# z430/keyword-spotting

Measured on AMD Instinct MI355X. Metric: 1s 16kHz clips/sec end-to-end (wav->label), higher is better.
Workload: dtype f32

## Files before the change

### keyword-spotting_amd/csrc/kws_dscnn.hip

```cpp
#include <array>
#include <utility>

#include "kws_dscnn_stages.h"

namespace kws {
namespace {

#ifndef KWS_X_DSCNN_STAMP_TID
#define KWS_X_DSCNN_STAMP_TID 0
#endif

__device__ __forceinline__ DscnnWeights weights_for_this_clip() {
#if defined(__HIP_DEVICE_COMPILE__)
    using KArg = const __attribute__((address_space(4))) DscnnWeights*;
    KArg p = (KArg)__builtin_amdgcn_kernarg_segment_ptr();
    asm volatile("" : "+s"(p));
    return *p;
#else
    return DscnnWeights{};
#endif
}

using FwdKernelFn = void (*)(DscnnWeights, const float*, int, float*, int32_t*, float*, unsigned long long*, const int*, StreamPush);
struct FwdKernelArgs {
// ... 58 lines not shown
        if (i < IN_T * IN_F) featp[(i / IN_F + 2) * FEAT_W + (i % IN_F) + 2] = fv[k];
    }
    if constexpr (PAIR) {
        float m = 0.f;
#pragma unroll
        for (int k = 0; k < FV; ++k) m = fmaxf(m, fabsf(fv[k]));
        publish_wave_max(lds, 0, wv, lane, m);
        if (lane == 63) lds[OFF_WMAX + wv + STAGE_WAVES] = 0.f;
    }
}

__device__ __forceinline__ void pool_fc_wave(const DscnnWeights& w, const float* lds, int lane, int clip, float* __restrict__ logits,
                                             int32_t* __restrict__ label, float* __restrict__ a_pool) {
    const int C = w.num_classes;
    float4 fcw[CH / 4];
    float fcb = 0.f;
    const float4* wr = reinterpret_cast<const float4*>(w.fc_w + (lane < C ? lane : 0) * CH);
#pragma unroll
    for (int c = 0; c < CH / 4; ++c) fcw[c] = wr[c];
    if (lane < C) fcb = w.fc_b[lane];
    const float ring_b = w.pw_b[3 * CH + lane];
    constexpr float RING_N = 55.f * 11.f - 53.f * 9.f;
    float s = 0.f;
#pragma unroll
    for (int k = 0; k < NW; ++k) s += lds[OFF_POOLBUF_P + k * CH + lane];
    s = fmaf(RING_N, relu(ring_b), s) * (1.0f / (55.f * 11.f));
    if (a_pool) a_pool[lane] = s;
    float acc = fcb;
#pragma unroll
    for (int c = 0; c < CH / 4; ++c) {
        const float4 a4 = fcw[c];
        acc = fmaf(a4.x, __builtin_bit_cast(float, __builtin_amdgcn_readlane(__builtin_bit_cast(int, s), 4 * c + 0)), acc);
        acc = fmaf(a4.y, __builtin_bit_cast(float, __builtin_amdgcn_readlane(__builtin_bit_cast(int, s), 4 * c + 1)), acc);
        acc = fmaf(a4.z, __builtin_bit_cast(float, __builtin_amdgcn_readlane(__builtin_bit_cast(int, s), 4 * c + 2)), acc);
        acc = fmaf(a4.w, __builtin_bit_cast(float, __builtin_amdgcn_readlane(__builtin_bit_cast(int, s), 4 * c + 3)), acc);
    }
    if (lane < C) logits[(size_t)clip * C + lane] = acc;
    const int idx = wave_argmax_first(lane < C ? acc : -INFINITY, lane, C);
    if (label && lane == 0) label[clip] = idx;
}

template <int MODE, bool DIAG = true, bool PRECONV = false, bool STREAM = false, bool CLUSTER = false, bool PERSIST = false,
          bool SCAN = false>
__global__ __launch_bounds__(NT) void kws_dscnn_fwd_kernel(DscnnWeights w_arg, const float* __restrict__ feat, int B,
                                                           float* __restrict__ logits, int32_t* __restrict__ label,
                                                           float* __restrict__ act_arg,
                                                           unsigned long long* __restrict__ stamps_arg,
                                                           const int* __restrict__ ring_hops, StreamPush sp) {
    static_assert(!STREAM || (MODE >= 4 && !DIAG && !PRECONV), "the fused push exists for the product paths only");
    static_assert(!PERSIST || ((MODE == 4 || MODE == 5) && !PRECONV && !STREAM), "persistent workgroups: batched product paths only");
    static_assert(!SCAN || ((MODE == 4 || MODE == 5) && !DIAG && !PRECONV && !STREAM && !CLUSTER), "strided windows: batched product paths only");
    constexpr bool PAIR = MODE == 5;
    constexpr int NP = PAIR ? 2 : 3;
    BlockTables t1_pre{};
    static_assert(!CLUSTER || STREAM, "time-tile clusters exist for the streaming push only");
    float* const act = DIAG ? act_arg : nullptr;
    unsigned long long* const stamps = DIAG ? stamps_arg : nullptr;
    extern __shared__ __attribute__((aligned(16))) float lds[];
    constexpr bool MFMA = MODE != 0;
    const int tid_k = threadIdx.x;
    const int lane_k = tid_k & 63, wv_k = tid_k >> 6;

    const int cl_n = CLUSTER ? sp.cluster : 1;
    int clip = CLUSTER ? (int)blockIdx.x / cl_n : (int)blockIdx.x;
    const int cl_tile = CLUSTER ? (int)blockIdx.x - clip * cl_n : 0;
    if (clip >= B) return;
    const int j0 = Blk<4>::H * cl_tile / cl_n, j1 = Blk<4>::H * (cl_tile + 1) / cl_n;
    auto rows = [&](int lo, int hi, int H, int W) { return PosRange{(lo < 0 ? 0 : lo) * W, (hi > H ? H : hi) * W}; };
    const PosRange rg4 = rows(j0, j1, Blk<4>::H, Blk<4>::W), rg3 = rows(j0 - 2, j1, Blk<3>::H, Blk<3>::W),
                   rg2 = rows(j0 - 4, j1, Blk<2>::H, Blk<2>::W), rg1 = rows(j0 - 6, j1, Blk<1>::H, Blk<1>::W),
                   rg0 = rows(j0 - 7, j1 + 1, C1_H, C1_W);
    int n_stamp = 0;
    auto stamp = [&]() {
        if (stamps && tid_k == KWS_X_DSCNN_STAMP_TID) stamps[(size_t)clip * KWS_DSCNN_STAMPS + n_stamp] = __builtin_amdgcn_s_memtime();
        ++n_stamp;
    };

    constexpr bool SPLIT = MODE >= 4;
    constexpr bool UT = PERSIST && PAIR;
    BlockTables t1p{};
    uintx4 c1p[PERSIST ? 7 : 1][NP];
    int prev_clip = -1;
    float* a_prev = nullptr;
    if constexpr (PERSIST) {
        fetch_block_tables(w_arg, 1, tid_k, t1p);
        if (wv_k < STAGE_WAVES) stage_features_persist<PAIR, SCAN>(lds, feat, clip, tid_k, sp.scan);
        load_conv1_frags(w_arg, wv_k, lane_k, c1p);
        __syncthreads();
    }
    for (;;) {
    auto weights_now = [&]() -> DscnnWeights { return PERSIST ? weights_for_this_clip() : w_arg; };
    const DscnnWeights w = weights_now();
    int tid = tid_k;
    if constexpr (PERSIST) {
        int wv_l = __builtin_amdgcn_readfirstlane(wv_k), lane_l = lane_k;
        asm volatile("" : "+s"(wv_l), "+v"(lane_l));
        tid = (wv_l << 6) | (lane_l & 63);
    }
    const int lane = tid & 63, wv = tid >> 6;
    if constexpr (PERSIST) n_stamp = 0;
    if (stamps && tid == KWS_X_DSCNN_STAMP_TID) stamps[(size_t)clip * KWS_DSCNN_STAMPS + KWS_DSCNN_STAMPS - 2] = __builtin_amdgcn_s_memrealtime();
    stamp();

    PwOperands<MODE> wa;
    UnitDesc ud{};
    int hops_before = 0;
    int kx = 0, ky[5] = {0, 0, 0, 0, 0}, sg[5] = {0, 0, 0, 0, 0};
    if constexpr (PERSIST) {
        if constexpr (PAIR) {
            const float mxf = read_stage_max(lds, 0, 1);
            kx = pow2_exp_for(mxf);
            const float bz0 = (w.c1_abs * mxf + w.c1_bmax) * 1.001f;
            cap_units(kx, sg[0], w.k_c1, bz0);
            const float by1 = (w.dw_abs[0] * bz0 + w.dw_bmax[0]) * 1.001f;
            ky[1] = pow2_exp_for(by1);
            cap_units(ky[1], sg[1], w.k_pw[0], (w.pw_abs[0] * by1 + w.pw_bmax[0]) * 1.001f);
            store_block_tables(lds, 1, tid, t1p, pow2f(ky[1]), pow2f(sg[1]), pow2f(ky[1] - sg[0]));
            conv1_build_windows(lds, tid, pow2f(kx), OFF_FEAT_P);
            __syncthreads();
        } else {
            store_block_tables(lds, 1, tid, t1p);
        }
        stamp();
        conv1_phase_split<false, NP>(w, lds, tid, c1p, rg0, pow2f(kx), pow2f(sg[0]), OFF_FEAT_P);
        if (wv == NW - 1 && prev_clip >= 0) {
            pool_fc_wave(w, lds, lane, prev_clip, logits, label, a_prev);
            if (stamps && lane == 0) stamps[(size_t)prev_clip * KWS_DSCNN_STAMPS + 13] = __builtin_amdgcn_s_memtime();
        }
        if constexpr (UT) load_unit_desc(w, 1, wv < Leftover<1>::TILE ? wv : Leftover<1>::TILE, lane, ud);
        load_afrag(w, 1, wv >= 4 ? wv - 4 : 0, lane, wa.ring[0]);
    } else if constexpr (PRECONV) {
        static_assert(!PRECONV || MODE >= 4, "the pre-convolved entry exists for the product (split) path only");
        const float* z = feat + (size_t)clip * (CH * P0);
        fetch_block_tables(w, 1, tid, t1_pre);
        float zmax = 0.f;
        for (int i = tid; i < CH * P0; i += NT) {
            const float v = z[i];
            lds[OFF_Z0 + pidx(i / P0, i % P0, P0 + 2)] = v;
            zmax = fmaxf(zmax, v);
        }
        if (tid < CH) {
            lds[OFF_Z0 + pidx(tid, P0, P0 + 2)] = 0.f;
            lds[OFF_Z0 + pidx(tid, P0 + 1, P0 + 2)] = 0.f;
        }
        if constexpr (PAIR)
            publish_wave_max(lds, 1, wv, lane, zmax);
        else
            store_block_tables(lds, 1, tid, t1_pre);
        if constexpr (Leftover<1>::HAS && (MODE == 4 || MODE == 5) && !CLUSTER)
            load_afrag(w, 1, wv >= 4 ? wv - 4 : 0, lane, wa.ring[0]);
        else
            load_block_head(w, 1, lane, wa);
        stamp();
    } else {
    float* featp = lds + OFF_FEAT;
    const float* f = clip_features<SCAN>(feat, clip, sp.scan);
    constexpr int FV = (IN_T * IN_F + NT - 1) / NT;
    float fv[FV];
    int row_new = -1;
    int head;
    if constexpr (STREAM) {
        hops_before = *sp.hops;
        const int K = frames_lag(sp.p);
        head = (((hops_before + 2 - K) % IN_T) + IN_T) % IN_T;
        const int step = sp.p.frame_step;
        const long f_start = (long)step * hops_before + step - (long)K * step;
// ... 12 lines not shown
    float a1[SPLIT ? 1 : 50];
    uintx4 c1f[SPLIT ? 7 : 1][NP];
    if constexpr (SPLIT) {
        load_conv1_frags(w, wv, lane, c1f);
    } else if constexpr (MFMA) {
        const int half = lane >> 5, col = lane & 31, ct = wv & 1;
#pragma unroll
        for (int s = 0; s < 50; ++s) a1[s] = w.c1_w[(2 * s + half) * CH + ct * 32 + col];
        load_pointwise(w, 1, lane, wa);
    }
    __builtin_amdgcn_sched_barrier(0);
    if constexpr (PAIR) {
        float m = 0.f;
#pragma unroll
        for (int k = 0; k < FV; ++k) m = fmaxf(m, fabsf(fv[k]));
        publish_wave_max(lds, 0, wv, lane, m);
    }
    if constexpr (STREAM) {
#ifdef KWS_X_STREAM_NO_FRAME
        if (false)
#else
        if (wv == 0 && cl_tile == cl_n - 1)
#endif
            stream_frame_wave(sp.p, sp.t, sp.hop, clip, clip, false, sp.pcm_ring, sp.ring_len, const_cast<float*>(feat), hops_before,
                              reinterpret_cast<unsigned char*>(lds + OFF_Z2), lane,
                              row_new >= 0 ? featp + (row_new + 2) * FEAT_W + 2 : nullptr, sp.refine_ctr);
        for (int i = tid; i < FEAT_H * FEAT_W; i += NT) {
            const int r = i / FEAT_W - 2, c = i % FEAT_W - 2;
            if (!((unsigned)r < (unsigned)IN_T && (unsigned)c < (unsigned)IN_F)) featp[i] = 0.f;
        }
        if constexpr (!PAIR) store_block_tables(lds, 1, tid, t1);
#pragma unroll
        for (int k = 0; k < FV; ++k) {
            const int i = tid + k * NT;
            if (i < IN_T * IN_F && i / IN_F != row_new) featp[(i / IN_F + 2) * FEAT_W + (i % IN_F) + 2] = fv[k];
        }
        __syncthreads();
    } else {
    for (int i = tid; i < FEAT_H * FEAT_W; i += NT) {
        const int r = i / FEAT_W - 2, c = i % FEAT_W - 2;
        if (!((unsigned)r < (unsigned)IN_T && (unsigned)c < (unsigned)IN_F)) featp[i] = 0.f;
    }
    if constexpr (!PAIR) store_block_tables(lds, 1, tid, t1);
#pragma unroll
    for (int k = 0; k < FV; ++k) {
        const int i = tid + k * NT;
        if (i < IN_T * IN_F) featp[(i / IN_F + 2) * FEAT_W + (i % IN_F) + 2] = fv[k];
    }
    __syncthreads();
    }
    if constexpr (PAIR) {
        float mxf = read_stage_max(lds, 0, 1);
        if constexpr (STREAM) {
            if (row_new >= 0 && cl_tile == cl_n - 1)
                for (int c = 0; c < IN_F; ++c) mxf = fmaxf(mxf, fabsf(featp[(row_new + 2) * FEAT_W + 2 + c]));
        }
        kx = pow2_exp_for(mxf);
        const float bz0 = (w.c1_abs * mxf + w.c1_bmax) * 1.001f;
        cap_units(kx, sg[0], w.k_c1, bz0);
        const float by1 = (w.dw_abs[0] * bz0 + w.dw_bmax[0]) * 1.001f;
        ky[1] = pow2_exp_for(by1);
        cap_units(ky[1], sg[1], w.k_pw[0], (w.pw_abs[0] * by1 + w.pw_bmax[0]) * 1.001f);
        store_block_tables(lds, 1, tid, t1, pow2f(ky[1]), pow2f(sg[1]), pow2f(ky[1] - sg[0]));
        conv1_build_windows(lds, tid, pow2f(kx));
        __syncthreads();
    }
    stamp();

    if constexpr (SPLIT) {
        conv1_phase_split<CLUSTER, NP>(w, lds, tid, c1f, rg0, pow2f(kx), pow2f(sg[0]));
        if constexpr (Leftover<1>::HAS && (MODE == 4 || MODE == 5) && !CLUSTER)
            load_afrag(w, 1, wv >= 4 ? wv - 4 : 0, lane, wa.ring[0]);
        else
            load_block_head(w, 1, lane, wa);
    } else {
        conv1_phase<MFMA>(w, lds, tid, a1);
    }
    }
    stamp();
    const DscnnWeights w1 = weights_now();
    __syncthreads();
    stamp();
    float* a = act ? act + (size_t)clip * KWS_ACT_FLOATS_PER_CLIP : nullptr;
    constexpr bool KSL_ON = (MODE == 4 || MODE == 5) && !CLUSTER;
    if (a) {
        const float u = PAIR ? pow2f(-sg[0]) : 1.f;
        for (int i = tid; i < CH * P0; i += NT) a[i] = lds[OFF_Z0 + pidx(i / P0, i % P0, P0 + 2)] * u;
        a += CH * P0;
    }
    PairCtx pc;
    if constexpr (PAIR && PRECONV) {
        const float mz0 = read_stage_max(lds, 1, 1);
        const float by1 = (w1.dw_abs[0] * mz0 + w1.dw_bmax[0]) * 1.001f;
        ky[1] = pow2_exp_for(by1);
        cap_units(ky[1], sg[1], w1.k_pw[0], (w1.pw_abs[0] * by1 + w1.pw_bmax[0]) * 1.001f);
        store_block_tables(lds, 1, tid, t1_pre, pow2f(ky[1]), pow2f(sg[1]), pow2f(ky[1]));
        __syncthreads();
    }
    if constexpr (PAIR) {
        const float mz = read_stage_max(lds, 1, 1) * pow2f(-sg[0]);
        const float bz = (w1.pw_abs[0] * ((w1.dw_abs[0] * mz + w1.dw_bmax[0]) * 1.001f) + w1.pw_bmax[0]) * 1.001f;
        const float by = (w1.dw_abs[1] * bz + w1.dw_bmax[1]) * 1.001f;
        ky[2] = pow2_exp_for(by);
        cap_units(ky[2], sg[2], w1.k_pw[1], (w1.pw_abs[1] * by + w1.pw_bmax[1]) * 1.001f);
        pc.s_dww = pow2f(ky[2] - sg[1]);
        pc.s_dwb = pow2f(ky[2]);
        pc.s_pwb = pow2f(sg[2]);
    }
    block_phase<1, MODE, CLUSTER, UT>(w1, lds, tid, wa, ud, nullptr, rg1, pc);
    stamp();
    const DscnnWeights w2 = weights_now();
    __syncthreads();
    if constexpr (Leftover<1>::HAS && KSL_ON) {
        leftover_combine<1, PAIR>(lds, tid);
        __syncthreads();
    }
    stamp();
    if (a) {
        const float u = PAIR ? pow2f(-sg[1]) : 1.f;
        for (int i = tid; i < CH * Blk<1>::POUT; i += NT)
            a[i] = lds[OFF_Z1 + pidx(i / Blk<1>::POUT, i % Blk<1>::POUT, Blk<1>::SOUT)] * u;
        a += CH * Blk<1>::POUT;
    }
    if constexpr (PAIR) {
        const float mz = fmaxf(read_stage_max(lds, 2, (Leftover<1>::HAS && KSL_ON) ? 2 : 1) * pow2f(-sg[1]), w2.pw_bmax[0]);
        const float bz = (w2.pw_abs[1] * ((w2.dw_abs[1] * mz + w2.dw_bmax[1]) * 1.001f) + w2.pw_bmax[1]) * 1.001f;
        const float by = (w2.dw_abs[2] * bz + w2.dw_bmax[2]) * 1.001f;
        ky[3] = pow2_exp_for(by);
        cap_units(ky[3], sg[3], w2.k_pw[2], (w2.pw_abs[2] * by + w2.pw_bmax[2]) * 1.001f);
        pc.s_dww = pow2f(ky[3] - sg[2]);
        pc.s_dwb = pow2f(ky[3]);
        pc.s_pwb = pow2f(sg[3]);
    }
    block_phase<2, MODE, CLUSTER, UT>(w2, lds, tid, wa, ud, nullptr, rg2, pc);
    stamp();
    const DscnnWeights w3 = weights_now();
    __syncthreads();
    if constexpr (Leftover<2>::HAS && KSL_ON) {
        leftover_combine<2, PAIR>(lds, tid);
        __syncthreads();
    }
    stamp();
    if (a) {
        const float u = PAIR ? pow2f(-sg[2]) : 1.f;
        for (int i = tid; i < CH * Blk<2>::POUT; i += NT)
            a[i] = lds[OFF_Z2 + pidx(i / Blk<2>::POUT, i % Blk<2>::POUT, Blk<2>::SOUT)] * u;
        a += CH * Blk<2>::POUT;
    }
    if constexpr (PAIR) {
        const float mz = fmaxf(read_stage_max(lds, 0, (Leftover<2>::HAS && KSL_ON) ? 2 : 1) * pow2f(-sg[2]), w3.pw_bmax[1]);
        const float bz = (w3.pw_abs[2] * ((w3.dw_abs[2] * mz + w3.dw_bmax[2]) * 1.001f) + w3.pw_bmax[2]) * 1.001f;
        const float by = (w3.dw_abs[3] * bz + w3.dw_bmax[3]) * 1.001f;
        ky[4] = pow2_exp_for(by);
        cap_units(ky[4], sg[4], w3.k_pw[3], (w3.pw_abs[3] * by + w3.pw_bmax[3]) * 1.001f);
        pc.s_dww = pow2f(ky[4] - sg[3]);
        pc.s_dwb = pow2f(ky[4]);
        pc.s_pwb = pow2f(sg[4]);
    }
    block_phase<3, MODE, CLUSTER, UT>(w3, lds, tid, wa, ud, nullptr, rg3, pc);
    stamp();
    const DscnnWeights w4 = weights_now();
    __syncthreads();
    stamp();
    if (a) {
        const float u = PAIR ? pow2f(-sg[3]) : 1.f;
        for (int i = tid; i < CH * Blk<3>::POUT; i += NT)
            a[i] = lds[OFF_Z3 + pidx(i / Blk<3>::POUT, i % Blk<3>::POUT, Blk<3>::SOUT)] * u;
        a += CH * Blk<3>::POUT;
    }
    if constexpr (PAIR) {
        pc.inv_out = pow2f(-sg[4]);
    }
    block_phase<4, MODE, CLUSTER, UT>(w4, lds, tid, wa, ud, a ? a + CH : nullptr, rg4, pc,
                                      PERSIST ? OFF_POOLBUF_P : OFF_POOLBUF);
    stamp();
    if constexpr (PERSIST) {
        const int next = clip + (int)gridDim.x;
        __builtin_amdgcn_sched_barrier(0);
        const ScanWindows sw_next = SCAN ? scan_windows_now() : ScanWindows{};
        if (wv < STAGE_WAVES && next < B) stage_features_persist<PAIR, SCAN>(lds, feat, next, tid, sw_next);
        stamp();
        load_conv1_frags(w4, wv, lane, c1p);
        __syncthreads();
        stamp();
        if (stamps && tid == KWS_X_DSCNN_STAMP_TID) stamps[(size_t)clip * KWS_DSCNN_STAMPS + KWS_DSCNN_STAMPS - 1] = __builtin_amdgcn_s_memrealtime();
        prev_clip = clip;
        a_prev = a;
        clip = next;
        if (clip >= B) break;
        continue;
    }
    const int C = w4.num_classes;
    float4 fcw[CH / 4];
    float fcb = 0.f, ring_b = 0.f;
    if (wv == 0 && lane < C) {
        const float4* wr = reinterpret_cast<const float4*>(w4.fc_w + lane * CH);
#pragma unroll
        for (int c = 0; c < CH / 4; ++c) fcw[c] = wr[c];
        fcb = w4.fc_b[lane];
    }
    if (tid < CH) ring_b = w4.pw_b[3 * CH + tid];
    __syncthreads();
    stamp();

    float* pooled = lds + OFF_POOLED;
    constexpr float RING_N = 55.f * 11.f - 53.f * 9.f;
    bool run_fc = true;
    if constexpr (CLUSTER) {
        float* part = sp.cl_part + ((size_t)clip * cl_n + cl_tile) * CH;
        if (tid < CH) {
            float s = 0.f;
#pragma unroll
            for (int k = 0; k < NW; ++k) s += lds[OFF_POOLBUF + k * CH + tid];
            __hip_atomic_store(part + tid, s, __ATOMIC_RELAXED, __HIP_MEMORY_SCOPE_AGENT);
        }
        asm volatile("s_waitcnt vmcnt(0)" ::: "memory");
        __syncthreads();
        int* last_flag = reinterpret_cast<int*>(lds + OFF_POOLED + CH);
        if (tid == 0) {
            const int arrived = atomicAdd(&sp.cl_count[clip], 1);
            *last_flag = arrived == cl_n - 1;
            if (arrived == cl_n - 1) sp.cl_count[clip] = 0;
        }
        __syncthreads();
        run_fc = *last_flag != 0;
        if (run_fc) {
            if (tid < CH) {
                float s = 0.f;
                for (int t = 0; t < cl_n; ++t)
                    s += __hip_atomic_load(sp.cl_part + ((size_t)clip * cl_n + t) * CH + tid, __ATOMIC_RELAXED, __HIP_MEMORY_SCOPE_AGENT);
                pooled[tid] = fmaf(RING_N, relu(ring_b), s) * (1.0f / (55.f * 11.f));
            }
        }
// ... 162 lines not shown
```

### keyword-spotting_amd/csrc/kws_dscnn_geom.h

```cpp
#pragma once
#include "kws_internal.h"

namespace kws {
namespace {

#ifndef KWS_DSCNN_WAVES
#define KWS_DSCNN_WAVES 8
#endif
constexpr int NW = KWS_DSCNN_WAVES;
constexpr int NT = NW * 64;
constexpr int TW = 30;

constexpr int P0 = C1_H * C1_W;
constexpr int FEAT_H = 103, FEAT_W = 14;
constexpr int OFF_Z3 = 0, OFF_Z2 = 22976, OFF_Z1 = 0, OFF_Z0 = 9152, OFF_FEAT = 18304;
constexpr int OFF_DWTAB = 38784;
constexpr int OFF_PWB = OFF_DWTAB + 2 * 768;
constexpr int OFF_POOLED = OFF_PWB + 2 * 64;
constexpr int OFF_POOLBUF = OFF_DWTAB;
constexpr int OFF_WMAX = OFF_POOLED + 64 + 8;
constexpr int LDS_FLOATS = 40960;
static_assert(OFF_WMAX + 4 * NW <= LDS_FLOATS, "LDS overflow");
static_assert(NW * 64 <= 768, "pool scratch must fit one depthwise buffer");
static_assert(OFF_FEAT + FEAT_H * FEAT_W <= OFF_Z2, "feature pad overlaps Z2");
static_assert(CH * 12 <= 2 * NT, "table staging assumes at most two elements per thread");

__host__ __device__ __forceinline__ constexpr int pidx(int c, int p, int S) { return (c >> 1) * 2 * S + 2 * p + (c & 1); }

template <int N>
struct Blk {
    static constexpr int H = 45 + 2 * N, W = 1 + 2 * N;
    static constexpr bool RING = N > 1;
    static constexpr int HI = RING ? H - 2 : H, WI = RING ? W - 2 : W;
    static constexpr int PIN = HI * WI, SIN = PIN + 2;
    static constexpr int POUT = H * W, SOUT = POUT + 2;
    static constexpr int OFF_IN = N == 1 ? OFF_Z0 : N == 2 ? OFF_Z1 : N == 3 ? OFF_Z2 : OFF_Z3;
    static constexpr int OFF_OUT = N == 1 ? OFF_Z1 : N == 2 ? OFF_Z2 : OFF_Z3;
    static constexpr int TILES = (POUT + TW - 1) / TW;
    static constexpr int BUF = (N - 1) & 1;
};

#ifndef KWS_DSCNN_KSPLIT_LEFTOVER
#define KWS_DSCNN_KSPLIT_LEFTOVER 1
#endif
template <int N>
struct Leftover {
    static constexpr bool HAS = KWS_DSCNN_KSPLIT_LEFTOVER && (N == 1 || N == 2);
    static constexpr int TILE = N == 1 ? 4 : 8;
    static constexpr int P0T = TILE * TW;
    static constexpr int NP = HAS ? Blk<N>::POUT - P0T : 1;
    static constexpr int WAVE0 = N == 1 ? 4 : 0;
    static constexpr int OFF_PART = N == 1 ? OFF_Z2 : OFF_Z0;
};
static_assert(Blk<1>::TILES == 5 && Blk<2>::TILES == 9, "the leftover tiles are the fifth of block 1 and the ninth of block 2");
static_assert(4 * CH * Leftover<1>::NP <= 38784 - OFF_Z2 && OFF_Z0 + 4 * CH * Leftover<2>::NP <= OFF_FEAT, "partial sums fit their dead planes");

constexpr int OFF_FEAT_P = OFF_Z2;
constexpr int OFF_POOLBUF_P = OFF_FEAT_P + 1456;
constexpr int STAGE_WAVES = 4;
static_assert(OFF_FEAT_P >= OFF_Z3 + Blk<3>::SOUT * CH, "the next clip's features must not overlap block 4's input");
static_assert(OFF_FEAT_P + FEAT_H * FEAT_W <= OFF_POOLBUF_P && OFF_POOLBUF_P % 4 == 0, "features and pool partials are disjoint");
static_assert(OFF_POOLBUF_P + NW * CH <= OFF_Z2 + Blk<2>::SOUT * CH && OFF_Z2 + Blk<2>::SOUT * CH <= OFF_DWTAB,
              "pool partials stay inside the Z2 plane, clear of the table buffers the next clip's block 1 rewrites");

}
}
```

### keyword-spotting_amd/csrc/kws_dscnn_stages.h

```cpp
#pragma once
#include <type_traits>

#include "kws_dscnn_geom.h"
#include "kws_dscnn_units.h"
#include "kws_mfcc_dev.h"
#include "kws_split_mfma.h"

namespace kws {
namespace {

template <bool TO_MFMA = false>
__device__ __forceinline__ float stencil3x3(float w0, float w1, float w2, float w3, float w4, float w5, float w6,
                                            float w7, float w8, float b, float up, float mid, float dn, float mask_l,
                                            float mask_r) {
    float c, to_right, to_left;
    asm("v_mul_f32 %1, %3, %13\n\t"
        "v_mul_f32 %2, %5, %13\n\t"
        "v_fma_f32 %0, %4, %13, %12\n\t"
        "v_fmac_f32 %1, %6, %14\n\t"
        "v_fmac_f32 %2, %8, %14\n\t"
        "v_fmac_f32 %0, %7, %14\n\t"
        "v_fmac_f32 %1, %9, %15\n\t"
        "v_fmac_f32 %2, %11, %15\n\t"
        "v_fmac_f32 %0, %10, %15\n\t"
// ... 420 lines not shown
            conv1_unit_pairwin<true>(w, lds, z0, wv, wv & 1, lane, c1f, 0, P0, sig0, mx);
        else if (wv < 6)
            conv1_unit_pairwin<false>(w, lds, z0, 4, wv & 1, lane, c1f, 0, P0, sig0, mx);
    } else if constexpr (RANGED) {
        const int n_pt = (rg.hi - rg.lo + 31) / 32;
        for (int u = wv; u < 2 * n_pt; u += NW) conv1_unit_split<false, NP>(w, featp, z0, u >> 1, u & 1, lane, c1f, rg.lo, rg.hi, sx, sig0, mx);
    } else if (wv < 4)
        conv1_unit_split<true, NP>(w, featp, z0, wv, wv & 1, lane, c1f, 0, P0, sx, sig0, mx);
    else if (wv < 6)
        conv1_unit_split<false, NP>(w, featp, z0, 4, wv & 1, lane, c1f, 0, P0, sx, sig0, mx);
    if constexpr (NP == 2) publish_wave_max(lds, 1, wv, lane, mx);
    if (tid < CH) {
        z0[pidx(tid, P0, P0 + 2)] = 0.f;
        z0[pidx(tid, P0 + 1, P0 + 2)] = 0.f;
    }
}

template <int N, int NP, bool UT = false>
__device__ __forceinline__ void leftover_partial_unit(float* lds, int lane, int M, const uintx4 (&af)[2][NP], const UnitDesc& ud) {
    using G = Blk<N>;
    using L = Leftover<N>;
    const int half = lane >> 5, col = lane & 31;
    const float* dwtab = lds + OFF_DWTAB + G::BUF * 768;
    const float4* dwt4 = reinterpret_cast<const float4*>(dwtab) + half * 24;
    bool valid;
    float mask_l, mask_r;
    int ta[3];
    if constexpr (UT) {
        valid = ud.a[3] != 0u;
        mask_l = __builtin_bit_cast(float, ud.m.x), mask_r = __builtin_bit_cast(float, ud.m.y);
#pragma unroll
        for (int i = 0; i < 3; ++i) ta[i] = (int)ud.a[i];
    } else {
        const int pos = L::P0T - 1 + col;
        valid = col >= 1 && col <= TW && pos < G::POUT;
        const int posc = pos < G::POUT ? pos : G::POUT - 1;
        const int h = posc / G::W, x = posc % G::W;
        mask_l = x > 0 ? 1.f : 0.f, mask_r = x < G::W - 1 ? 1.f : 0.f;
#pragma unroll
        for (int dh = -1; dh <= 1; ++dh) {
            const int o = G::RING ? 1 : 0;
            const int hh = h + dh - o, xx = x - o;
            const bool inside = (unsigned)hh < (unsigned)G::HI && (unsigned)xx < (unsigned)G::WI;
            const bool in_map = (unsigned)(h + dh) < (unsigned)G::H;
            const int a = inside ? hh * G::WI + xx : ((G::RING && in_map) ? G::PIN : G::PIN + 1);
            ta[dh + 1] = G::OFF_IN + pidx(half * 8, a, G::SIN);
        }
    }
    float y[8];
#pragma unroll
    for (int j = 0; j < 8; j += 2) {
        const int cs = 16 * M + j;
        const int o = cs * G::SIN;
        const float2 up = *reinterpret_cast<const float2*>(lds + ta[0] + o);
        const float2 mid = *reinterpret_cast<const float2*>(lds + ta[1] + o);
        const float2 dn = *reinterpret_cast<const float2*>(lds + ta[2] + o);
        DwPair wp;
#pragma unroll
        for (int i = 0; i < 5; ++i) wp.l[i] = dwt4[(cs >> 1) * 6 + i];
        y[j] = stencil3x3_of_pair<false, 0>(wp, up.x, mid.x, dn.x, mask_l, mask_r);
        y[j + 1] = stencil3x3_of_pair<false, 1>(wp, up.y, mid.y, dn.y, mask_l, mask_r);
    }
    floatx16 acc0 = {0, 0, 0, 0, 0, 0, 0, 0, 0, 0, 0, 0, 0, 0, 0, 0}, acc1 = acc0;
    if constexpr (NP == 2) {
        uintx4 bh, bl;
        split_pair8_scaled(y, bh, bl);
        acc0 = mfma_f16(af[0][0], bl, acc0);
        acc1 = mfma_f16(af[1][0], bl, acc1);
        acc0 = mfma_f16(af[0][1], bh, acc0);
        acc1 = mfma_f16(af[1][1], bh, acc1);
        acc0 = mfma_f16(af[0][0], bh, acc0);
        acc1 = mfma_f16(af[1][0], bh, acc1);
    } else {
        uintx4 bh, bm, bl;
        split3(y, bh, bm, bl);
#pragma unroll
        for (int q = 0; q < 6; ++q) {
            const int pa = q == 0 ? 2 : (q == 2 || q == 3) ? 1 : 0;
            const uintx4& b = (q == 0 || q == 3 || q == 5) ? bh : (q == 1 ? bl : bm);
            acc0 = mfma_bf16(af[0][pa], b, acc0);
            acc1 = mfma_bf16(af[1][pa], b, acc1);
        }
    }
    float* part = lds + L::OFF_PART + M * (CH * L::NP);
    if (valid) {
#pragma unroll
        for (int r = 0; r < 16; ++r) {
            part[row_of(r, half) * L::NP + (col - 1)] = acc0[r];
            part[(32 + row_of(r, half)) * L::NP + (col - 1)] = acc1[r];
        }
    }
}

template <int N, bool PAIR = false>
__device__ __forceinline__ void leftover_combine(float* lds, int tid) {
    using G = Blk<N>;
    using L = Leftover<N>;
    const float* part = lds + L::OFF_PART;
    const float* pwb = lds + OFF_PWB + G::BUF * 64;
    float* zout = lds + G::OFF_OUT;
    float mx = 0.f;
    for (int i = tid; i < CH * L::NP; i += NT) {
        const int co = i / L::NP, j = i - co * L::NP;
        const float s = (part[i] + part[CH * L::NP + i]) + (part[2 * CH * L::NP + i] + part[3 * CH * L::NP + i]);
        const float v = relu(s + pwb[co]);
        zout[pidx(co, L::P0T + j, G::SOUT)] = v;
        mx = fmaxf(mx, v);
    }
    if constexpr (PAIR) publish_wave_max(lds, N == 1 ? 3 : 1, tid >> 6, tid & 63, mx);
}

template <int N, int MODE, bool RANGED = false, bool UT = false>
__device__ __forceinline__ void block_phase(const DscnnWeights& w, float* lds, int tid, PwOperands<MODE>& pwo, UnitDesc& ud,
                                            float* __restrict__ act4 = nullptr, PosRange rg = PosRange{0, 0}, PairCtx pc = PairCtx{},
                                            int off_poolbuf = OFF_POOLBUF) {
    static_assert(!UT || ((MODE == 4 || MODE == 5) && !RANGED && Leftover<1>::HAS), "unit descriptors: product paths on whole maps");
    using G = Blk<N>;
    constexpr bool PAIR = MODE == 5;
    constexpr int NP = PAIR ? 2 : 3;
    constexpr int NPROD = PAIR ? 3 : 6;
    constexpr bool KSL = Leftover<N>::HAS && (MODE == 4 || MODE == 5) && !RANGED;
    const int p_lo = RANGED ? rg.lo : 0, p_hi = RANGED ? rg.hi : G::POUT;
#ifdef KWS_X_DSCNN_SKIP_LEFTOVER
    const int n_tiles = RANGED ? (p_hi - p_lo + TW - 1) / TW : (N == 2 ? 8 : G::TILES);
#else
    const int n_tiles = RANGED ? (p_hi - p_lo + TW - 1) / TW : (KSL ? Leftover<N>::TILE : G::TILES);
#endif
    constexpr bool MFMA = MODE != 0;
    constexpr bool SPLIT = MODE >= 4;
    constexpr bool NO_STENCIL = MODE == 6;
    const int lane = tid & 63, wv = tid >> 6, half = lane >> 5, col = lane & 31;
    float* zout = lds + G::OFF_OUT;
    const float* dwtab = lds + OFF_DWTAB + G::BUF * 768;
    const float* pwb = lds + OFF_PWB + G::BUF * 64;
    float* poolbuf = lds + off_poolbuf;

    BlockTables next_tables;
    if constexpr (N < 4) {
        fetch_block_tables(w, N + 1, tid, next_tables);
        if (tid < CH) {
            zout[pidx(tid, G::POUT, G::SOUT)] = relu(pwb[tid]);
            zout[pidx(tid, G::POUT + 1, G::SOUT)] = 0.f;
        }
    } else if (!MFMA) {
        poolbuf[wv * CH + lane] = 0.f;
    }

    const float4* bias4 = reinterpret_cast<const float4*>(pwb) + half;
    const float4* dwt4 = reinterpret_cast<const float4*>(dwtab) + half * 24;
    float psum[2][16];
#pragma unroll
    for (int ct = 0; ct < 2; ++ct)
#pragma unroll
        for (int r = 0; r < 16; ++r) psum[ct][r] = 0.f;
    float stage_max = 0.f;

    for (int t = wv; t < n_tiles; t += NW) {
        const int pos = p_lo + t * TW - 1 + col;
        bool valid;
        uint32_t keep;
        float mask_l, mask_r;
        int tlo[3], thi[3];
        if constexpr (UT) {
            keep = ud.a[3];
            valid = keep != 0u;
            mask_l = __builtin_bit_cast(float, ud.m.x), mask_r = __builtin_bit_cast(float, ud.m.y);
#pragma unroll
            for (int i = 0; i < 3; ++i) {
                tlo[i] = (int)ud.a[i];
                thi[i] = tlo[i] + 32 * G::SIN;
                asm volatile("" : "+v"(tlo[i]));
                asm volatile("" : "+v"(thi[i]));
            }
        } else {
            valid = col >= 1 && col <= TW && pos < p_hi;
            keep = valid ? 0xffffffffu : 0u;
            const int posc = pos < p_lo ? p_lo : (pos < p_hi ? pos : p_hi - 1);
            const int h = posc / G::W, x = posc % G::W;
            mask_l = x > 0 ? 1.f : 0.f, mask_r = x < G::W - 1 ? 1.f : 0.f;
#pragma unroll
            for (int dh = -1; dh <= 1; ++dh) {
                const int o = G::RING ? 1 : 0;
                const int hh = h + dh - o, xx = x - o;
                const bool inside = (unsigned)hh < (unsigned)G::HI && (unsigned)xx < (unsigned)G::WI;
                const bool in_map = (unsigned)(h + dh) < (unsigned)G::H;
                const int a = inside ? hh * G::WI + xx : ((G::RING && in_map) ? G::PIN : G::PIN + 1);
                tlo[dh + 1] = G::OFF_IN + pidx(half * 8, a, G::SIN);
                thi[dh + 1] = tlo[dh + 1] + 32 * G::SIN;
                asm volatile("" : "+v"(tlo[dh + 1]));
                asm volatile("" : "+v"(thi[dh + 1]));
            }
        }
// ... 150 lines not shown
                        }
#pragma unroll
                        for (int r = 0; r < 16; r += 2) stage_max = fmaxf(stage_max, fmaxf(fmaxf(o0[r], o0[r + 1]), fmaxf(o1[r], o1[r + 1])));
                        if (valid) {
#pragma unroll
                            for (int r = 0; r < 16; r += 2) {
                                *reinterpret_cast<float2*>(zout + pidx(row_of(r, half), pos, G::SOUT)) = make_float2(o0[r], o0[r + 1]);
                                *reinterpret_cast<float2*>(zout + pidx(32 + row_of(r, half), pos, G::SOUT)) = make_float2(o1[r], o1[r + 1]);
                            }
                        }
                    } else if (valid) {
#pragma unroll
                        for (int r = 0; r < 16; r += 2) {
                            *reinterpret_cast<float2*>(zout + pidx(row_of(r, half), pos, G::SOUT)) =
                                make_float2(relu(acc0[r]), relu(acc0[r + 1]));
                            *reinterpret_cast<float2*>(zout + pidx(32 + row_of(r, half), pos, G::SOUT)) =
                                make_float2(relu(acc1[r]), relu(acc1[r + 1]));
                        }
                    }
                } else {
#pragma unroll
                    for (int r = 0; r < 16; ++r) {
                        psum[0][r] += __builtin_bit_cast(float, __builtin_bit_cast(uint32_t, relu(acc0[r])) & keep);
                        psum[1][r] += __builtin_bit_cast(float, __builtin_bit_cast(uint32_t, relu(acc1[r])) & keep);
                    }
                    if (act4 && valid) {
#pragma unroll
                        for (int r = 0; r < 16; ++r) {
                            act4[row_of(r, half) * G::POUT + pos] = relu(acc0[r]) * pc.inv_out;
                            act4[(32 + row_of(r, half)) * G::POUT + pos] = relu(acc1[r]) * pc.inv_out;
                        }
                    }
                }
            };
            if constexpr (!SPLIT) {
                if (N < 4 && t + NW >= n_tiles) {
                    __builtin_amdgcn_sched_barrier(0);
                    if constexpr (N < 4) load_pointwise(w, N + 1, lane, pwo);
                    __builtin_amdgcn_sched_barrier(0);
                    epilogue();
                    break;
                }
            }
            epilogue();
            if constexpr (UT) ud = ud_next;
        } else {
            const float* pw_w = w.pw_w + (N - 1) * CH * CH;
            float y[32];
#pragma unroll
            for (int s = 0; s < 32; s += 2) {
                TapPair tq;
                tap_pair_load(s >> 1, tq);
                DwPair wp;
                wts_pair_load(s >> 1, wp);
                y[s] = dw_eval(wp, tq, std::integral_constant<int, 0>{});
                y[s + 1] = dw_eval(wp, tq, std::integral_constant<int, 1>{});
            }
#pragma unroll 1
            for (int co = 0; co < CH; ++co) {
                float part = 0.f;
#pragma unroll
                for (int s = 0; s < 32; ++s) part = fmaf(pw_w[(16 * (s >> 3) + 8 * half + (s & 7)) * CH + co], y[s], part);
                const float tot = relu(part + __shfl_xor(part, 32, 64) + pwb[co]);
                if constexpr (N < 4) {
                    if (valid && half == 0) zout[pidx(co, pos, G::SOUT)] = tot;
                } else {
                    if (act4 && valid && half == 0) act4[co * G::POUT + pos] = tot;
                    float sum = (valid && half == 0) ? tot : 0.f;
#pragma unroll
                    for (int o = 16; o >= 1; o >>= 1) sum += __shfl_xor(sum, o, 64);
                    if (lane == 0) poolbuf[wv * CH + co] += sum;
                }
            }
        }
    }

    if constexpr (KSL) {
        using L = Leftover<N>;
        if (wv >= L::WAVE0 && wv < L::WAVE0 + 4) {
            leftover_partial_unit<N, NP, UT>(lds, lane, wv - L::WAVE0, pwo.ring[0], ud);
            __builtin_amdgcn_sched_barrier(0);
            if constexpr (UT) load_unit_desc(w, N + 1, wv, lane, ud);
            load_afrag(w, N + 1, 0, lane, pwo.ring[0]);
        }
    }
    if constexpr (N < 4) store_block_tables(lds, N + 1, tid, next_tables, pc.s_dwb, pc.s_pwb, pc.s_dww);
    if constexpr (PAIR && N <= 2) publish_wave_max(lds, N == 1 ? 2 : 0, wv, lane, stage_max);
    if constexpr (MFMA) {
        if constexpr (N < 4) {
            if (wv >= n_tiles && !(KSL && N == 1)) load_block_head(w, N + 1, lane, pwo);
        } else {
#pragma unroll
            for (int ct = 0; ct < 2; ++ct) {
                float (&q)[16] = psum[ct];
                asm volatile("s_nop 4\n\t"
                    "v_add_f32_dpp %0, %0, %0 row_shr:1 row_mask:0xf bank_mask:0xf bound_ctrl:1\n\t"
                    "v_add_f32_dpp %1, %1, %1 row_shr:1 row_mask:0xf bank_mask:0xf bound_ctrl:1\n\t"
                    "v_add_f32_dpp %2, %2, %2 row_shr:1 row_mask:0xf bank_mask:0xf bound_ctrl:1\n\t"
                    "v_add_f32_dpp %3, %3, %3 row_shr:1 row_mask:0xf bank_mask:0xf bound_ctrl:1\n\t"
                    "v_add_f32_dpp %4, %4, %4 row_shr:1 row_mask:0xf bank_mask:0xf bound_ctrl:1\n\t"
                    "v_add_f32_dpp %5, %5, %5 row_shr:1 row_mask:0xf bank_mask:0xf bound_ctrl:1\n\t"
                    "v_add_f32_dpp %6, %6, %6 row_shr:1 row_mask:0xf bank_mask:0xf bound_ctrl:1\n\t"
                    "v_add_f32_dpp %7, %7, %7 row_shr:1 row_mask:0xf bank_mask:0xf bound_ctrl:1\n\t"
                    "v_add_f32_dpp %8, %8, %8 row_shr:1 row_mask:0xf bank_mask:0xf bound_ctrl:1\n\t"
                    "v_add_f32_dpp %9, %9, %9 row_shr:1 row_mask:0xf bank_mask:0xf bound_ctrl:1\n\t"
                    "v_add_f32_dpp %10, %10, %10 row_shr:1 row_mask:0xf bank_mask:0xf bound_ctrl:1\n\t"
                    "v_add_f32_dpp %11, %11, %11 row_shr:1 row_mask:0xf bank_mask:0xf bound_ctrl:1\n\t"
                    "v_add_f32_dpp %12, %12, %12 row_shr:1 row_mask:0xf bank_mask:0xf bound_ctrl:1\n\t"
                    "v_add_f32_dpp %13, %13, %13 row_shr:1 row_mask:0xf bank_mask:0xf bound_ctrl:1\n\t"
                    "v_add_f32_dpp %14, %14, %14 row_shr:1 row_mask:0xf bank_mask:0xf bound_ctrl:1\n\t"
                    "v_add_f32_dpp %15, %15, %15 row_shr:1 row_mask:0xf bank_mask:0xf bound_ctrl:1\n\t"
                    "v_add_f32_dpp %0, %0, %0 row_shr:2 row_mask:0xf bank_mask:0xf bound_ctrl:1\n\t"
                    "v_add_f32_dpp %1, %1, %1 row_shr:2 row_mask:0xf bank_mask:0xf bound_ctrl:1\n\t"
                    "v_add_f32_dpp %2, %2, %2 row_shr:2 row_mask:0xf bank_mask:0xf bound_ctrl:1\n\t"
                    "v_add_f32_dpp %3, %3, %3 row_shr:2 row_mask:0xf bank_mask:0xf bound_ctrl:1\n\t"
                    "v_add_f32_dpp %4, %4, %4 row_shr:2 row_mask:0xf bank_mask:0xf bound_ctrl:1\n\t"
                    "v_add_f32_dpp %5, %5, %5 row_shr:2 row_mask:0xf bank_mask:0xf bound_ctrl:1\n\t"
                    "v_add_f32_dpp %6, %6, %6 row_shr:2 row_mask:0xf bank_mask:0xf bound_ctrl:1\n\t"
                    "v_add_f32_dpp %7, %7, %7 row_shr:2 row_mask:0xf bank_mask:0xf bound_ctrl:1\n\t"
                    "v_add_f32_dpp %8, %8, %8 row_shr:2 row_mask:0xf bank_mask:0xf bound_ctrl:1\n\t"
                    "v_add_f32_dpp %9, %9, %9 row_shr:2 row_mask:0xf bank_mask:0xf bound_ctrl:1\n\t"
                    "v_add_f32_dpp %10, %10, %10 row_shr:2 row_mask:0xf bank_mask:0xf bound_ctrl:1\n\t"
                    "v_add_f32_dpp %11, %11, %11 row_shr:2 row_mask:0xf bank_mask:0xf bound_ctrl:1\n\t"
                    "v_add_f32_dpp %12, %12, %12 row_shr:2 row_mask:0xf bank_mask:0xf bound_ctrl:1\n\t"
                    "v_add_f32_dpp %13, %13, %13 row_shr:2 row_mask:0xf bank_mask:0xf bound_ctrl:1\n\t"
                    "v_add_f32_dpp %14, %14, %14 row_shr:2 row_mask:0xf bank_mask:0xf bound_ctrl:1\n\t"
                    "v_add_f32_dpp %15, %15, %15 row_shr:2 row_mask:0xf bank_mask:0xf bound_ctrl:1\n\t"
                    "v_add_f32_dpp %0, %0, %0 row_shr:4 row_mask:0xf bank_mask:0xf bound_ctrl:1\n\t"
                    "v_add_f32_dpp %1, %1, %1 row_shr:4 row_mask:0xf bank_mask:0xf bound_ctrl:1\n\t"
                    "v_add_f32_dpp %2, %2, %2 row_shr:4 row_mask:0xf bank_mask:0xf bound_ctrl:1\n\t"
                    "v_add_f32_dpp %3, %3, %3 row_shr:4 row_mask:0xf bank_mask:0xf bound_ctrl:1\n\t"
                    "v_add_f32_dpp %4, %4, %4 row_shr:4 row_mask:0xf bank_mask:0xf bound_ctrl:1\n\t"
                    "v_add_f32_dpp %5, %5, %5 row_shr:4 row_mask:0xf bank_mask:0xf bound_ctrl:1\n\t"
                    "v_add_f32_dpp %6, %6, %6 row_shr:4 row_mask:0xf bank_mask:0xf bound_ctrl:1\n\t"
                    "v_add_f32_dpp %7, %7, %7 row_shr:4 row_mask:0xf bank_mask:0xf bound_ctrl:1\n\t"
                    "v_add_f32_dpp %8, %8, %8 row_shr:4 row_mask:0xf bank_mask:0xf bound_ctrl:1\n\t"
                    "v_add_f32_dpp %9, %9, %9 row_shr:4 row_mask:0xf bank_mask:0xf bound_ctrl:1\n\t"
                    "v_add_f32_dpp %10, %10, %10 row_shr:4 row_mask:0xf bank_mask:0xf bound_ctrl:1\n\t"
                    "v_add_f32_dpp %11, %11, %11 row_shr:4 row_mask:0xf bank_mask:0xf bound_ctrl:1\n\t"
                    "v_add_f32_dpp %12, %12, %12 row_shr:4 row_mask:0xf bank_mask:0xf bound_ctrl:1\n\t"
                    "v_add_f32_dpp %13, %13, %13 row_shr:4 row_mask:0xf bank_mask:0xf bound_ctrl:1\n\t"
                    "v_add_f32_dpp %14, %14, %14 row_shr:4 row_mask:0xf bank_mask:0xf bound_ctrl:1\n\t"
                    "v_add_f32_dpp %15, %15, %15 row_shr:4 row_mask:0xf bank_mask:0xf bound_ctrl:1\n\t"
                    "v_add_f32_dpp %0, %0, %0 row_shr:8 row_mask:0xf bank_mask:0xf bound_ctrl:1\n\t"
                    "v_add_f32_dpp %1, %1, %1 row_shr:8 row_mask:0xf bank_mask:0xf bound_ctrl:1\n\t"
                    "v_add_f32_dpp %2, %2, %2 row_shr:8 row_mask:0xf bank_mask:0xf bound_ctrl:1\n\t"
                    "v_add_f32_dpp %3, %3, %3 row_shr:8 row_mask:0xf bank_mask:0xf bound_ctrl:1\n\t"
                    "v_add_f32_dpp %4, %4, %4 row_shr:8 row_mask:0xf bank_mask:0xf bound_ctrl:1\n\t"
                    "v_add_f32_dpp %5, %5, %5 row_shr:8 row_mask:0xf bank_mask:0xf bound_ctrl:1\n\t"
                    "v_add_f32_dpp %6, %6, %6 row_shr:8 row_mask:0xf bank_mask:0xf bound_ctrl:1\n\t"
                    "v_add_f32_dpp %7, %7, %7 row_shr:8 row_mask:0xf bank_mask:0xf bound_ctrl:1\n\t"
                    "v_add_f32_dpp %8, %8, %8 row_shr:8 row_mask:0xf bank_mask:0xf bound_ctrl:1\n\t"
                    "v_add_f32_dpp %9, %9, %9 row_shr:8 row_mask:0xf bank_mask:0xf bound_ctrl:1\n\t"
                    "v_add_f32_dpp %10, %10, %10 row_shr:8 row_mask:0xf bank_mask:0xf bound_ctrl:1\n\t"
                    "v_add_f32_dpp %11, %11, %11 row_shr:8 row_mask:0xf bank_mask:0xf bound_ctrl:1\n\t"
                    "v_add_f32_dpp %12, %12, %12 row_shr:8 row_mask:0xf bank_mask:0xf bound_ctrl:1\n\t"
                    "v_add_f32_dpp %13, %13, %13 row_shr:8 row_mask:0xf bank_mask:0xf bound_ctrl:1\n\t"
                    "v_add_f32_dpp %14, %14, %14 row_shr:8 row_mask:0xf bank_mask:0xf bound_ctrl:1\n\t"
                    "v_add_f32_dpp %15, %15, %15 row_shr:8 row_mask:0xf bank_mask:0xf bound_ctrl:1\n\t"
                    "v_add_f32_dpp %0, %0, %0 row_bcast:15 row_mask:0xa bank_mask:0xf\n\t"
                    "v_add_f32_dpp %1, %1, %1 row_bcast:15 row_mask:0xa bank_mask:0xf\n\t"
                    "v_add_f32_dpp %2, %2, %2 row_bcast:15 row_mask:0xa bank_mask:0xf\n\t"
                    "v_add_f32_dpp %3, %3, %3 row_bcast:15 row_mask:0xa bank_mask:0xf\n\t"
                    "v_add_f32_dpp %4, %4, %4 row_bcast:15 row_mask:0xa bank_mask:0xf\n\t"
                    "v_add_f32_dpp %5, %5, %5 row_bcast:15 row_mask:0xa bank_mask:0xf\n\t"
                    "v_add_f32_dpp %6, %6, %6 row_bcast:15 row_mask:0xa bank_mask:0xf\n\t"
// ... 45 lines not shown
```

Baseline: 7.388 million.

## Fold leftover-tile combine into last-arriving wave via LDS atomic counter

Replaces the separate leftover_combine pass, which needed an extra workgroup barrier after blocks 1 and 2, with a last-arriver scheme. Each of the four partial-sum waves bumps an LDS atomic counter, and the fourth wave alone reduces the partials, adds bias and applies ReLU. Partials are now stored as float4 in a padded channel-major layout so the combine can use vector loads. This removes two __syncthreads per clip, but the combine now runs on one wave instead of all waves and depends on LDS atomic ordering being correct.

```diff
diff --git a/keyword-spotting_amd/csrc/kws_dscnn.hip b/keyword-spotting_amd/csrc/kws_dscnn.hip
--- a/keyword-spotting_amd/csrc/kws_dscnn.hip
+++ b/keyword-spotting_amd/csrc/kws_dscnn.hip
@@ -164,6 +164,7 @@
     uintx4 c1p[PERSIST ? 7 : 1][NP];
     int prev_clip = -1;
     float* a_prev = nullptr;
+    if ((MODE == 4 || MODE == 5) && !CLUSTER && tid_k == 0) lds[OFF_ARRIVE] = 0.f;
     if constexpr (PERSIST) {
         fetch_block_tables(w_arg, 1, tid_k, t1p);
         if (wv_k < STAGE_WAVES) stage_features_persist<PAIR, SCAN>(lds, feat, clip, tid_k, sp.scan);
@@ -342,7 +343,6 @@
     __syncthreads();
     stamp();
     float* a = act ? act + (size_t)clip * KWS_ACT_FLOATS_PER_CLIP : nullptr;
-    constexpr bool KSL_ON = (MODE == 4 || MODE == 5) && !CLUSTER;
     if (a) {
         const float u = PAIR ? pow2f(-sg[0]) : 1.f;
         for (int i = tid; i < CH * P0; i += NT) a[i] = lds[OFF_Z0 + pidx(i / P0, i % P0, P0 + 2)] * u;
@@ -371,10 +371,6 @@
     stamp();
     const DscnnWeights w2 = weights_now();
     __syncthreads();
-    if constexpr (Leftover<1>::HAS && KSL_ON) {
-        leftover_combine<1, PAIR>(lds, tid);
-        __syncthreads();
-    }
     stamp();
     if (a) {
         const float u = PAIR ? pow2f(-sg[1]) : 1.f;
@@ -383,7 +379,7 @@
         a += CH * Blk<1>::POUT;
     }
     if constexpr (PAIR) {
-        const float mz = fmaxf(read_stage_max(lds, 2, (Leftover<1>::HAS && KSL_ON) ? 2 : 1) * pow2f(-sg[1]), w2.pw_bmax[0]);
+        const float mz = fmaxf(read_stage_max(lds, 2, 1) * pow2f(-sg[1]), w2.pw_bmax[0]);
         const float bz = (w2.pw_abs[1] * ((w2.dw_abs[1] * mz + w2.dw_bmax[1]) * 1.001f) + w2.pw_bmax[1]) * 1.001f;
         const float by = (w2.dw_abs[2] * bz + w2.dw_bmax[2]) * 1.001f;
         ky[3] = pow2_exp_for(by);
@@ -396,10 +392,6 @@
     stamp();
     const DscnnWeights w3 = weights_now();
     __syncthreads();
-    if constexpr (Leftover<2>::HAS && KSL_ON) {
-        leftover_combine<2, PAIR>(lds, tid);
-        __syncthreads();
-    }
     stamp();
     if (a) {
         const float u = PAIR ? pow2f(-sg[2]) : 1.f;
@@ -408,7 +400,7 @@
         a += CH * Blk<2>::POUT;
     }
     if constexpr (PAIR) {
-        const float mz = fmaxf(read_stage_max(lds, 0, (Leftover<2>::HAS && KSL_ON) ? 2 : 1) * pow2f(-sg[2]), w3.pw_bmax[1]);
+        const float mz = fmaxf(read_stage_max(lds, 0, 1) * pow2f(-sg[2]), w3.pw_bmax[1]);
         const float bz = (w3.pw_abs[2] * ((w3.dw_abs[2] * mz + w3.dw_bmax[2]) * 1.001f) + w3.pw_bmax[2]) * 1.001f;
         const float by = (w3.dw_abs[3] * bz + w3.dw_bmax[3]) * 1.001f;
         ky[4] = pow2_exp_for(by);
diff --git a/keyword-spotting_amd/csrc/kws_dscnn_geom.h b/keyword-spotting_amd/csrc/kws_dscnn_geom.h
--- a/keyword-spotting_amd/csrc/kws_dscnn_geom.h
+++ b/keyword-spotting_amd/csrc/kws_dscnn_geom.h
@@ -19,8 +19,9 @@
 constexpr int OFF_POOLED = OFF_PWB + 2 * 64;
 constexpr int OFF_POOLBUF = OFF_DWTAB;
 constexpr int OFF_WMAX = OFF_POOLED + 64 + 8;
+constexpr int OFF_ARRIVE = OFF_WMAX + 3 * NW;
 constexpr int LDS_FLOATS = 40960;
-static_assert(OFF_WMAX + 4 * NW <= LDS_FLOATS, "LDS overflow");
+static_assert(OFF_ARRIVE + 1 <= LDS_FLOATS, "LDS overflow");
 static_assert(NW * 64 <= 768, "pool scratch must fit one depthwise buffer");
 static_assert(OFF_FEAT + FEAT_H * FEAT_W <= OFF_Z2, "feature pad overlaps Z2");
 static_assert(CH * 12 <= 2 * NT, "table staging assumes at most two elements per thread");
@@ -51,9 +52,12 @@
     static constexpr int NP = HAS ? Blk<N>::POUT - P0T : 1;
     static constexpr int WAVE0 = N == 1 ? 4 : 0;
     static constexpr int OFF_PART = N == 1 ? OFF_Z2 : OFF_Z0;
+    static constexpr int CSTRIDE = CH + 4;
+    static constexpr int PART = NP * CSTRIDE;
 };
 static_assert(Blk<1>::TILES == 5 && Blk<2>::TILES == 9, "the leftover tiles are the fifth of block 1 and the ninth of block 2");
-static_assert(4 * CH * Leftover<1>::NP <= 38784 - OFF_Z2 && OFF_Z0 + 4 * CH * Leftover<2>::NP <= OFF_FEAT, "partial sums fit their dead planes");
+static_assert(4 * Leftover<1>::PART <= 38784 - OFF_Z2 && OFF_Z0 + 4 * Leftover<2>::PART <= OFF_FEAT, "partial sums fit their dead planes");
+static_assert(Leftover<1>::OFF_PART % 4 == 0 && Leftover<2>::OFF_PART % 4 == 0 && Leftover<1>::CSTRIDE % 4 == 0, "partial sums move as float4s");
 
 constexpr int OFF_FEAT_P = OFF_Z2;
 constexpr int OFF_POOLBUF_P = OFF_FEAT_P + 1456;
diff --git a/keyword-spotting_amd/csrc/kws_dscnn_stages.h b/keyword-spotting_amd/csrc/kws_dscnn_stages.h
--- a/keyword-spotting_amd/csrc/kws_dscnn_stages.h
+++ b/keyword-spotting_amd/csrc/kws_dscnn_stages.h
@@ -526,32 +526,61 @@
             acc1 = mfma_bf16(af[1][pa], b, acc1);
         }
     }
-    float* part = lds + L::OFF_PART + M * (CH * L::NP);
     if (valid) {
-#pragma unroll
-        for (int r = 0; r < 16; ++r) {
-            part[row_of(r, half) * L::NP + (col - 1)] = acc0[r];
-            part[(32 + row_of(r, half)) * L::NP + (col - 1)] = acc1[r];
-        }
-    }
-}
-
-template <int N, bool PAIR = false>
-__device__ __forceinline__ void leftover_combine(float* lds, int tid) {
+        float4* part4 = reinterpret_cast<float4*>(lds + L::OFF_PART + M * L::PART + (col - 1) * L::CSTRIDE) + half;
+#pragma unroll
+        for (int q = 0; q < 4; ++q) {
+            part4[2 * q] = make_float4(acc0[4 * q], acc0[4 * q + 1], acc0[4 * q + 2], acc0[4 * q + 3]);
+            part4[8 + 2 * q] = make_float4(acc1[4 * q], acc1[4 * q + 1], acc1[4 * q + 2], acc1[4 * q + 3]);
+        }
+    }
+}
+
+template <int N>
+__device__ __forceinline__ float leftover_arrive(float* lds, int lane) {
     using G = Blk<N>;
     using L = Leftover<N>;
-    const float* part = lds + L::OFF_PART;
-    const float* pwb = lds + OFF_PWB + G::BUF * 64;
-    float* zout = lds + G::OFF_OUT;
+    int* arrived = reinterpret_cast<int*>(lds + OFF_ARRIVE);
+    asm volatile("s_waitcnt lgkmcnt(0)" ::: "memory");
+    int before = 0;
+    if (lane == 0) before = __hip_atomic_fetch_add(arrived, 1, __ATOMIC_RELAXED, __HIP_MEMORY_SCOPE_WORKGROUP);
+    before = __builtin_amdgcn_readfirstlane(before);
+    asm volatile("" ::: "memory");
     float mx = 0.f;
-    for (int i = tid; i < CH * L::NP; i += NT) {
-        const int co = i / L::NP, j = i - co * L::NP;
-        const float s = (part[i] + part[CH * L::NP + i]) + (part[2 * CH * L::NP + i] + part[3 * CH * L::NP + i]);
-        const float v = relu(s + pwb[co]);
-        zout[pidx(co, L::P0T + j, G::SOUT)] = v;
-        mx = fmaxf(mx, v);
-    }
-    if constexpr (PAIR) publish_wave_max(lds, N == 1 ? 3 : 1, tid >> 6, tid & 63, mx);
+    if (before == 3) {
+        const float4* part4 = reinterpret_cast<const float4*>(lds + L::OFF_PART);
+        float* zout = lds + G::OFF_OUT;
+        const int cq = lane & 15;
+        const float4 b = reinterpret_cast<const float4*>(lds + OFF_PWB + G::BUF * 64)[cq];
+        constexpr int ROUNDS = (L::NP + 3) / 4, RB = 2;
+        static_assert(ROUNDS % RB == 0, "whole batches");
+        auto comb = [&](float p0, float p1, float p2, float p3, float bias) { return relu(((p0 + p1) + (p2 + p3)) + bias); };
+#pragma unroll 1
+        for (int r0 = 0; r0 < ROUNDS; r0 += RB) {
+            float4 p[RB][4];
+#pragma unroll
+            for (int r = 0; r < RB; ++r) {
+                const int j = (lane >> 4) + 4 * (r0 + r);
+                const int jc = j < L::NP ? j : L::NP - 1;
+#pragma unroll
+                for (int m = 0; m < 4; ++m) p[r][m] = part4[(m * L::PART + jc * L::CSTRIDE) / 4 + cq];
+            }
+#pragma unroll
+            for (int r = 0; r < RB; ++r) {
+                const int j = (lane >> 4) + 4 * (r0 + r);
+                const float4(&q)[4] = p[r];
+                const float v0 = comb(q[0].x, q[1].x, q[2].x, q[3].x, b.x), v1 = comb(q[0].y, q[1].y, q[2].y, q[3].y, b.y);
+                const float v2 = comb(q[0].z, q[1].z, q[2].z, q[3].z, b.z), v3 = comb(q[0].w, q[1].w, q[2].w, q[3].w, b.w);
+                if (j < L::NP) {
+                    *reinterpret_cast<float2*>(zout + pidx(4 * cq, L::P0T + j, G::SOUT)) = make_float2(v0, v1);
+                    *reinterpret_cast<float2*>(zout + pidx(4 * cq + 2, L::P0T + j, G::SOUT)) = make_float2(v2, v3);
+                    mx = fmaxf(mx, fmaxf(fmaxf(v0, v1), fmaxf(v2, v3)));
+                }
+            }
+        }
+        if (lane == 0) *arrived = 0;
+    }
+    return mx;
 }
 
 template <int N, int MODE, bool RANGED = false, bool UT = false>
@@ -868,6 +897,8 @@
             __builtin_amdgcn_sched_barrier(0);
             if constexpr (UT) load_unit_desc(w, N + 1, wv, lane, ud);
             load_afrag(w, N + 1, 0, lane, pwo.ring[0]);
+            __builtin_amdgcn_sched_barrier(0);
+            stage_max = fmaxf(stage_max, leftover_arrive<N>(lds, lane));
         }
     }
     if constexpr (N < 4) store_block_tables(lds, N + 1, tid, next_tables, pc.s_dwb, pc.s_pwb, pc.s_dww);
```

Result: faster. 7.513 million (median of 6 runs) (+1.7%).
